# JunFenngZhi/YOLO-Fastest-and-Embedded-deployment

Measured on NVIDIA B200. Metric: images/sec at 640x512 b256, 1/2/4/8 B200; % HBM roofline per kernel, higher is better.
Workload: dtype f32

## Files before the change

### yolo_fastest_b200/csrc/yf_api.cu

```cuda
#include <cuda_runtime.h>

#include <algorithm>
#include <cmath>
#include <cstdarg>
#include <cstdio>
#include <cstdlib>
#include <cstring>
#include <map>
#include <string>
#include <utility>
#include <vector>

#include "../../include/yf.h"
#include "yf_kernels.cuh"
#include "yf_post.cuh"
#include "yf_tc.cuh"
#include "yf_tct.cuh"
#include "yf_wirb.cuh"
#include "yf_tcpw.cuh"
#include "yf_tcup.cuh"
#include "yf_tcirb2.cuh"
#include "yf_tcdense.cuh"
#include "yf_tcdense2.cuh"
#include "yf_prep.cuh"

using namespace yf;

namespace {

struct Spec {
    std::string name;
    int cin, cout, k, groups;
    bool deconv;
    int64_t w_off, b_off;
    int64_t w_count() const { return deconv ? (int64_t)cin * cout * k * k : (int64_t)cout * (cin / groups) * k * k; }
};

struct SpecTable {
    std::vector<Spec> specs;
    std::map<std::string, int> index;
    int64_t total = 0;
    void add(const std::string& name, int cin, int cout, int k, int groups = 1, bool deconv = false) {
        Spec s{name, cin, cout, k, groups, deconv, 0, 0};
        s.w_off = total;
        total += s.w_count();
        s.b_off = total;
        total += cout;
        index[name] = (int)specs.size();
        specs.push_back(s);
    }
    void irb(const std::string& name, int io, int mid) {
        add(name + ".conv1", io, mid, 1);
        add(name + ".conv2", mid, mid, 3, mid);
        add(name + ".conv3", mid, io, 1);
    }
    const Spec& get(const std::string& name) const { return specs[index.at(name)]; }
};

int head_channels(int num_cls, int num_anchors, int variant) {
    return (variant == YF_VARIANT_LITE ? num_anchors * num_cls : num_anchors) * (5 + num_cls);
}

SpecTable build_specs(int in_ch, int num_cls, int num_anchors, int variant = 0) {
    SpecTable t;
    const int nout = head_channels(num_cls, num_anchors, variant);
    t.add("conv0", in_ch, 8, 3);
    t.add("conv1_2", 8, 8, 1); t.add("conv1_3", 8, 8, 3, 8); t.add("conv1_4", 8, 4, 1);
    t.irb("res1_1", 4, 8);
    t.add("conv1_8", 4, 24, 1); t.add("conv1_9", 24, 24, 3); t.add("conv2_1", 24, 8, 1);
    t.irb("res2_1", 8, 32); t.irb("res2_2", 8, 32);
    t.add("conv2_2", 8, 32, 1); t.add("conv2_3", 32, 32, 3, 32); t.add("conv3_1", 32, 8, 1);
    t.irb("res3_1", 8, 48); t.irb("res3_2", 8, 48);
    t.add("conv3_2", 8, 48, 1); t.add("conv3_3", 48, 48, 3, 48); t.add("conv3_4", 48, 16, 1);
    t.irb("res3_3", 16, 96); t.irb("res3_4", 16, 96); t.irb("res3_5", 16, 96); t.irb("res3_6", 16, 96);
    t.add("conv3_5", 16, 96, 1); t.add("conv3_6", 96, 96, 3, 96); t.add("conv4_1", 96, 24, 1);
    t.irb("res4_1", 24, 136); t.irb("res4_2", 24, 136); t.irb("res4_3", 24, 136); t.irb("res4_4", 24, 136);
    t.add("conv4_2", 24, 136, 1); t.add("conv4_3", 136, 136, 3, 136); t.add("conv5_1", 136, 48, 1);
    t.irb("res5_1", 48, 224); t.irb("res5_2", 48, 224); t.irb("res5_3", 48, 224); t.irb("res5_4", 48, 224);
    t.irb("res5_5", 48, 224);
    t.add("conv5_2", 48, 96, 1);
    t.add("conv5_3", 96, 96, 5, 96); t.add("conv5_4", 96, 128, 1);
    t.add("conv5_5", 128, 128, 5, 128); t.add("conv5_6", 128, 128, 1);
    t.add("head_5", 128, nout, 1);
    t.add("deconv5_1", 96, 96, 2, 1, true);
    t.add("conv4_1_1", 232, 96, 1);
    t.add("conv4_1_2", 96, 96, 5, 96); t.add("conv4_1_3", 96, 96, 1);
    t.add("conv4_1_4", 96, 96, 5, 96); t.add("conv4_1_5", 96, 96, 1);
    t.add("head_4", 96, nout, 1);
    return t;
}

thread_local std::string g_err;

void set_err(std::string* dst, const char* fmt, ...) {
    char buf[1024];
    va_list ap;
    va_start(ap, fmt);
    vsnprintf(buf, sizeof buf, fmt, ap);
    va_end(ap);
    (dst ? *dst : g_err) = buf;
}

}

struct TmaCache {
    CUtensorMap map;
    const void* ptr = nullptr;
    int B = 0;
    bool u8 = false;
    bool failed = false;
};

struct GroupArgs {
    TmaCache* tc = nullptr;
    int nsm = 148;
    int resident = 148;
    const float* x = nullptr;
    const float* x2 = nullptr;
    float* y = nullptr;
    float* skip = nullptr;
    const float* w = nullptr;
    const float* w2 = nullptr;
    const DenseSmall* small = nullptr;
    bool pdl = false;
    int Hin = 0, Win = 0, Hout = 0, Wout = 0;
    int headn = 0;
};

template <class... KA, class... A>
inline void launch_k(bool pdl, void (*kernel)(KA...), int grid, int block, size_t smem, cudaStream_t st, A&&... args) {
    cudaLaunchConfig_t cfg;
    memset(&cfg, 0, sizeof cfg);
    cfg.gridDim = dim3((unsigned)grid); cfg.blockDim = dim3((unsigned)block); cfg.dynamicSmemBytes = smem; cfg.stream = st;
    cudaLaunchAttribute at[1];
    at[0].id = cudaLaunchAttributeProgrammaticStreamSerialization;
    at[0].val.programmaticStreamSerializationAllowed = 1;
    cfg.attrs = at; cfg.numAttrs = pdl ? 1u : 0u;
    cudaLaunchKernelEx(&cfg, kernel, std::forward<A>(args)...);
}

struct Group {
    int (*occupancy)() = nullptr;
    const char* name;
    void (*launch)(const GroupArgs&, const void* xin, bool u8in, int B, cudaStream_t);
    GroupArgs a;
    int out_ch;
    int64_t w_off;
    TmaCache tcache;
};

struct yf_ctx {
    int variant = 0;
    int device = 0, in_ch = 1, num_cls = 3, num_anchors = 3, max_batch = 1, H = 0, W = 0;
    int nout = 0;
    bool weights_loaded = false;
    std::string err;
    SpecTable specs;
    std::vector<Group> groups;
    std::vector<float> host_packed;
    float* d_w = nullptr;
    std::vector<float*> d_act;
    std::map<std::string, std::pair<float*, int64_t>> taps;
    float* d_skip = nullptr;
    float* d_hl = nullptr;
    float* d_hs = nullptr;
    float* d_x = nullptr;
    unsigned char* d_u8 = nullptr;
    yf_det* d_out = nullptr;
    int out_cap = 0;
    int32_t* d_counts = nullptr;
    int32_t* d_status = nullptr;
    int NC = 0;
    yf_det* p_rec = nullptr;
    double* p_conf = nullptr;
    int32_t* p_cls = nullptr;
    int4* p_sbox = nullptr;
    int32_t* p_order = nullptr;
    unsigned char* p_alive = nullptr;
    cudaStream_t s_copy = nullptr, s_comp = nullptr, s_back = nullptr;
    cudaStream_t s_cap = nullptr;
    cudaStream_t s_side = nullptr;
    DenseSmall dense_small;
    bool last_forward_forked = false;
    cudaEvent_t ev_fork = nullptr, ev_join = nullptr;
    unsigned char* sl_u8[2] = {nullptr, nullptr};
    yf_det* sl_out[2] = {nullptr, nullptr};
    int sl_out_cap[2] = {0, 0};
    int32_t* sl_counts[2] = {nullptr, nullptr};
    int32_t* sl_status[2] = {nullptr, nullptr};
    cudaEvent_t sl_in[2] = {nullptr, nullptr}, sl_free[2] = {nullptr, nullptr}, sl_done[2] = {nullptr, nullptr};
    bool sl_used[2] = {false, false};
    std::map<std::string, std::pair<cudaGraphExec_t, int>> graphs;
    PrepTap* prep_tab = nullptr;
    int prep_Ho = 0, prep_Wo = 0;
    unsigned char* d_bgr = nullptr;
    size_t bgr_cap = 0;
    unsigned char* n_alive = nullptr;
    int n_alive_cap = 0;
    int64_t launches = 0;
};

#define CTX_CHECK(ctx)                                         \
    if (!(ctx)) { set_err(nullptr, "null ctx"); return YF_ERR_ARG; }
#define CU(call)                                                                              \
    do {                                                                                      \
        cudaError_t e__ = (call);                                                             \
        if (e__ != cudaSuccess) {                                                             \
            set_err(&ctx->err, "%s failed: %s (%s:%d)", #call, cudaGetErrorString(e__), __FILE__, __LINE__); \
            return YF_ERR_CUDA;                                                               \
        }                                                                                     \
    } while (0)

#ifndef YF_CFGSTEM
#define YF_CFGSTEM StemCfg<8, 80, 256, 2>
#endif
using CfgStem = YF_CFGSTEM;
using CfgStem3 = StemCfg<8, 40, 256, 2, 3>;
#ifndef YF_CFGRES1
#define YF_CFGRES1 IrbCfg<4, 8, 4, 3, 1, 8, 80, 8, 8, 4, 8, 256, 3, true, true, false, false>
#endif
using CfgRes1 = YF_CFGRES1;
#ifndef YF_USE_WIRB
#define YF_USE_WIRB 1
#endif
#ifndef YF_CFGRES1_W
#define YF_CFGRES1_W WirbCfg<4, 8, 4, 1, 4, 8, 6, 12, true, true>
#endif
using CfgRes1W = YF_CFGRES1_W;
#ifndef YF_CFGRES2_W
#define YF_CFGRES2_W WirbCfg<8, 32, 8, 1, 8, 2, 6, 12, true, false>
#endif
using CfgRes2W = YF_CFGRES2_W;
#ifndef YF_CFGDOWN2_W
#define YF_CFGDOWN2_W WirbCfg<8, 32, 8, 2, 4, 2, 8, 12, false, false>
#endif
using CfgDown2W = YF_CFGDOWN2_W;
#ifndef YF_CFGSTEM_W
#define YF_CFGSTEM_W WstemCfg<12>
#endif
using CfgStemW = YF_CFGSTEM_W;

#ifndef YF_CFGDENSE
#define YF_CFGDENSE DenseCfg<8, 40, 4, 128, 3, 2>
#endif
using CfgDense = YF_CFGDENSE;
#ifndef YF_CFGRES2
#define YF_CFGRES2 IrbCfg<8, 32, 8, 3, 1, 8, 40, 16, 8, 4, 8, 128, 4, true, true, false, false>
#endif
using CfgRes2 = YF_CFGRES2;
#ifndef YF_CFGDOWN2
#define YF_CFGDOWN2 IrbCfg<8, 32, 8, 3, 2, 4, 40, 8, 8, 4, 4, 128, 3, true, false, false, false>
#endif
using CfgDown2 = YF_CFGDOWN2;
#ifndef YF_CFGRES3A
#define YF_CFGRES3A IrbCfg<8, 48, 8, 3, 1, 8, 40, 16, 8, 4, 8, 128, 4, true, true, false, false>
#endif
using CfgRes3a = YF_CFGRES3A;
#ifndef YF_CFGWIDE3
#define YF_CFGWIDE3 IrbCfg<8, 48, 16, 3, 1, 8, 40, 24, 8, 8, 8, 256, 2, true, false, false, false>
#endif
using CfgWide3 = YF_CFGWIDE3;
#ifndef YF_CFGRES3B
#define YF_CFGRES3B IrbCfg<16, 96, 16, 3, 1, 8, 40, 16, 8, 8, 8, 256, 2, true, true, false, false>
#endif
using CfgRes3b = YF_CFGRES3B;
#ifndef YF_TC3_TH
#define YF_TC3_TH 8
#define YF_TC3_TW 40
#define YF_TC3_MC 32
#define YF_TC3_RH 8
#define YF_TC3_NWW 10
#endif
#ifndef YF_TC3_OCC
#define YF_TC3_OCC 1
#endif
#ifndef YF_TC3_E1ALL
#define YF_TC3_E1ALL false
#endif
#ifndef YF_CFGRES3B_TC
#define YF_CFGRES3B_TC IrbTcCfg<16, 96, 16, YF_TC3_TH, YF_TC3_TW, YF_TC3_MC, YF_TC3_RH, YF_TC3_NWW, true, YF_TC3_E1ALL, YF_TC3_OCC>
#endif
using CfgRes3bTc = YF_CFGRES3B_TC;
#ifndef YF_USE_TCT
#define YF_USE_TCT 1
#endif
#ifndef YF_USE_TCT_A
#define YF_USE_TCT_A 1
#endif
using CfgRes3bTt = IrbTtCfg<16, 96, 16, 16, true>;
using CfgRes4Tt = IrbTtCfg<24, 136, 24, 8, true, 2>;
#ifndef YF_TCT_A_TH
#define YF_TCT_A_TH 16
#define YF_TCT_A_OCC 1
#endif
using CfgRes3aTt = IrbTtCfg<8, 48, 8, YF_TCT_A_TH, true, 0, YF_TCT_A_OCC>;
using CfgWide3Tt = IrbTtCfg<8, 48, 16, YF_TCT_A_TH, false, 0, YF_TCT_A_OCC>;
using CfgDown3Tt = IrbTtCfg<16, 96, 24, 8, false, 0, 1, 2>;
using CfgDown4Tt = IrbTtCfg<24, 136, 48, 4, false, 1, 1, 2, true, true>;
#ifndef YF_CFGRES4_TC
#define YF_CFGRES4_TC IrbTcCfg<24, 136, 24, 8, 20, 32, 4, 10, true, true>
#endif
using CfgRes4Tc = YF_CFGRES4_TC;
#ifndef YF_USE_TC
#define YF_USE_TC 1
#endif
#ifndef YF_CFGDOWN3
#define YF_CFGDOWN3 IrbCfg<16, 96, 24, 3, 2, 4, 40, 16, 8, 8, 4, 256, 2, true, false, false, false>
#endif
using CfgDown3 = YF_CFGDOWN3;
#ifndef YF_CFGRES4
#define YF_CFGRES4 IrbCfg<24, 136, 24, 3, 1, 8, 40, 16, 8, 8, 8, 256, 2, true, true, false, false>
#endif
using CfgRes4 = YF_CFGRES4;
#ifndef YF_CFGDOWN4
#define YF_CFGDOWN4 IrbCfg<24, 136, 48, 3, 2, 2, 20, 16, 8, 8, 2, 128, 4, true, false, true, true>
#endif
using CfgDown4 = YF_CFGDOWN4;
#ifndef YF_CFGRES5
#define YF_CFGRES5 IrbCfg<48, 224, 48, 3, 1, 8, 20, 16, 8, 8, 8, 256, 2, true, true, false, false>
#endif
using CfgRes5 = YF_CFGRES5;
#ifndef YF_CFGPW52
#define YF_CFGPW52 PwCfg<48, 96, 80, 8, 256, true>
#endif
using CfgPw52 = YF_CFGPW52;
using CfgLite34 = PwPwCfg<8, 48, 16, 128>;
#ifndef YF_CFGNECKS1
#define YF_CFGNECKS1 IrbCfg<96, 96, 128, 5, 1, 8, 20, 48, 4, 8, 4, 640, 1, false, false, false, false>
#endif
using CfgNeckS1 = YF_CFGNECKS1;
#ifndef YF_CFGNECKS2
#define YF_CFGNECKS2 IrbCfg<128, 128, 128, 5, 1, 8, 20, 32, 4, 8, 4, 640, 1, false, false, false, false, 1>
#endif
using CfgNeckS2 = YF_CFGNECKS2;
#ifndef YF_CFGUPCAT
#define YF_CFGUPCAT UpCatCfg<8, 20, 16, 4, 256, 2>
#endif
using CfgUpCat = YF_CFGUPCAT;
#ifndef YF_CFGNECKL1
#define YF_CFGNECKL1 IrbCfg<96, 96, 96, 5, 1, 4, 40, 32, 4, 8, 4, 256, 2, false, false, false, false>
#endif
using CfgNeckL1 = YF_CFGNECKL1;
#ifndef YF_CFGNECKL2
#define YF_CFGNECKL2 IrbCfg<96, 96, 96, 5, 1, 4, 40, 16, 4, 8, 4, 256, 2, false, false, false, false, 1>
#endif
using CfgNeckL2 = YF_CFGNECKL2;
#ifndef YF_CFGNECKS1_TC
#define YF_CFGNECKS1_TC DwPwTcCfg<96, 128, 5, 16, 20, 16, 4, 10, false>
#endif
using CfgNeckS1Tc = YF_CFGNECKS1_TC;
#ifndef YF_CFGNECKL1_TC
#define YF_CFGNECKL1_TC DwPwTcCfg<96, 96, 5, 8, 40, 16, 4, 10, false>
#endif
using CfgNeckL1Tc = YF_CFGNECKL1_TC;
#ifndef YF_CFGNECKS2_TC
#define YF_CFGNECKS2_TC DwPwTcCfg<128, 32, 5, 16, 20, 16, 4, 10, false, true>
#endif
using CfgNeckS2Tc = YF_CFGNECKS2_TC;
#ifndef YF_CFGNECKL2_TC
#define YF_CFGNECKL2_TC DwPwTcCfg<96, 32, 5, 8, 40, 16, 4, 10, false, true>
#endif
using CfgNeckL2Tc = YF_CFGNECKL2_TC;
static bool heads_on_tc(int nout) { return YF_USE_TC && nout <= 32; }
using CfgUpCatTc = UpCatTcCfg<10>;
using CfgDenseTc = DenseTcCfg<12>;
#ifndef YF_DENSE_TC
#define YF_DENSE_TC YF_USE_TC
#endif
#ifndef YF_RES5_TC
#define YF_RES5_TC YF_USE_TC
#endif
#ifndef YF_CFGRES5_TC
#define YF_CFGRES5_TC IrbTc2Cfg<48, 224, 48, 8, 20, 2, 2, 10, true>
#endif
using CfgRes5Tc = YF_CFGRES5_TC;
using CfgRes5TcS = IrbTc2Cfg<48, 224, 48, 4, 20, 2, 2, 10, true>;
using CfgRes4TcS = IrbTcCfg<24, 136, 24, 4, 20, 32, 4, 10, true, true>;
using CfgRes3bTcS = IrbTcCfg<16, 96, 16, 4, 40, 32, 4, 10, true, YF_TC3_E1ALL>;
using CfgRes5TcXS = IrbTc2Cfg<48, 224, 48, 2, 20, 2, 2, 10, true>;
using CfgRes5TcN = IrbTc2Cfg<48, 224, 48, 8, 12, 2, 2, 10, true>;
using CfgNeckS1TcN = DwPwTcCfg<96, 128, 5, 8, 12, 16, 4, 10, false>;
using CfgNeckS2TcN = DwPwTcCfg<128, 32, 5, 8, 12, 16, 4, 10, false, true>;
using CfgNeckL1TcN = DwPwTcCfg<96, 96, 5, 8, 20, 16, 4, 10, false>;
using CfgNeckL2TcN = DwPwTcCfg<96, 32, 5, 8, 20, 16, 4, 10, false, true>;
using CfgDown3N = IrbCfg<16, 96, 24, 3, 2, 4, 20, 16, 8, 8, 4, 256, 2, true, false, false, false>;
using CfgDown4N = IrbCfg<24, 136, 48, 3, 2, 2, 12, 16, 8, 8, 2, 128, 4, true, false, true, true>;
using CfgNeckL1TcS = DwPwTcCfg<96, 96, 5, 4, 20, 16, 4, 10, false>;
using CfgNeckL2TcS = DwPwTcCfg<96, 32, 5, 4, 20, 16, 4, 10, false, true>;
using CfgNeckS1TcS = DwPwTcCfg<96, 128, 5, 4, 20, 16, 4, 10, false>;
using CfgNeckS2TcS = DwPwTcCfg<128, 32, 5, 4, 20, 16, 4, 10, false, true>;
using CfgRes3bTcXS = IrbTcCfg<16, 96, 16, 2, 40, 32, 2, 10, true, YF_TC3_E1ALL>;
using CfgRes4TcXS = IrbTcCfg<24, 136, 24, 2, 20, 32, 2, 10, true, true>;
static bool upcat_on_tc(int H, int W) { return YF_USE_TC && ((W / 16) % 4 == 0) && ((H / 16) % 2 == 0); }

namespace {

template <class C>
void launch_irb(const GroupArgs& g, const void*, bool, int B, cudaStream_t st) {
    using G = typename C::G;
    const int tx = cdiv(g.Wout, G::TW), ty = cdiv(g.Hout, G::TH);
    const int total = B * tx * ty;
    const int grid = total < g.resident ? total : g.resident;
    irb_kernel<C><<<grid, C::NT, C::SMEM_BYTES, st>>>(g.x, g.y, g.skip, g.w, g.Hin, g.Win, g.Hout, g.Wout, tx, ty, total, g.headn);
}
template <class CB, class CN>
void launch_irb_auto(const GroupArgs& g, const void* x, bool u8, int B, cudaStream_t st) {
    static_assert(CB::CB == CN::CB && CB::OFF_B2 == CN::OFF_B2 && CB::MC == CN::MC, "both tile shapes read the same packed weights");
    const int big = B * cdiv(g.Wout, CB::G::TW) * cdiv(g.Hout, CB::G::TH);
    if (g.Wout <= CN::G::TW || 2 * big <= g.nsm) launch_irb<CN>(g, x, u8, B, st);
    else launch_irb<CB>(g, x, u8, B, st);
}
template <class K>
int occ_of(K kernel, int nt, int smem) {
    int n = 0;
    if (cudaOccupancyMaxActiveBlocksPerMultiprocessor(&n, kernel, nt, smem) != cudaSuccess || n < 1) n = 1;
    return n;
}
template <class C> int occ_irb() { return occ_of(irb_kernel<C>, C::NT, C::SMEM_BYTES); }
int occ_stem() { return occ_of(stem_kernel<CfgStem, false>, CfgStem::NT, CfgStem::SMEM_BYTES); }
int occ_stem3() { return occ_of(stem_kernel<CfgStem3, false>, CfgStem3::NT, CfgStem3::SMEM_BYTES); }
int occ_dense() { return occ_of(dense_kernel<CfgDense>, CfgDense::NT, CfgDense::SMEM_BYTES); }
int occ_upcat() { return occ_of(upcat_kernel<CfgUpCat>, CfgUpCat::NT, CfgUpCat::SMEM_BYTES); }
int occ_upcat_tc() { return occ_of(upcat_tc_kernel<CfgUpCatTc>, CfgUpCatTc::NT, CfgUpCatTc::SMEM_BYTES); }
void launch_upcat_tc(const GroupArgs& g, const void*, bool, int B, cudaStream_t st) {
    using C = CfgUpCatTc;
    const int tx = cdiv(g.Wout, C::TW), ty = cdiv(g.Hout, C::TH);
    const int total = B * tx * ty;
    const int grid = total < g.resident ? total : g.resident;
    launch_k(g.pdl, upcat_tc_kernel<C>, grid, C::NT, C::SMEM_BYTES, st, g.x, g.x2, g.y, g.w, g.Hout, g.Wout, tx, ty, total);
}

template <class C>
int wirb_band_rows(int B, int Hout, int Wout, int warps) {
    const int nstrips = cdiv(Wout, C::OW);
    long long best_cost = -1;
    int best_R = 1;
    for (int nch = 1; nch <= 16; ++nch) {
        const int R = C::S == 1 ? nch * C::RC - 2 : (nch * C::RC - 1) / 2;
        if (R < 1) continue;
        const long long units = (long long)B * nstrips * cdiv(Hout, R);
        const long long cost = ((units + warps - 1) / warps) * (nch * C::RC + 2);
        if (best_cost < 0 || cost <= best_cost) { best_cost = cost; best_R = R; }
        if (R >= Hout) break;
    }
    return best_R;
}
template <class C>
void launch_wirb(const GroupArgs& g, const void*, bool, int B, cudaStream_t st) {
    TmaCache* tc = g.tc;
    if (tc->ptr != g.x || tc->B != B) {
        tc->failed = tma_make_map4(&tc->map, g.x, 4, B, C::CIN, g.Hin, g.Win, C::XW, C::RC, C::CIN) != 0;
        tc->ptr = g.x; tc->B = B;
    }
    if (g.Wout % C::SPX) tc->failed = true;
    if (tc->failed) return;
    const int R = wirb_band_rows<C>(B, g.Hout, g.Wout, g.nsm * C::NW);
    const int nstrips = cdiv(g.Wout, C::OW), nbands = cdiv(g.Hout, R);
    const int total = B * nstrips * nbands;
    const int grid = std::min(g.nsm, cdiv(total, C::NW));
    launch_k(g.pdl, wirb_kernel<C>, grid, C::NW * 32, C::SMEM_BYTES, st, tc->map, g.y, g.w, g.Hin, g.Win, g.Hout, g.Wout, R, nstrips, nbands, total);
}
template <class C>
void launch_wstem(const GroupArgs& g, const void* xin, bool u8in, int B, cudaStream_t st) {
    TmaCache* tc = g.tc;
    if (tc->ptr != xin || tc->B != B || tc->u8 != u8in) {
        tc->failed = (u8in ? tma_make_map4(&tc->map, xin, 1, B, 1, g.Hin, g.Win, C::RAWWU, C::RAWH, 1)
                           : tma_make_map4(&tc->map, xin, 4, B, 1, g.Hin, g.Win, C::RAWW, C::RAWH, 1)) != 0;
        tc->ptr = xin; tc->B = B; tc->u8 = u8in;
    }
    if (g.Wout % C::SPX) tc->failed = true;
    if (tc->failed) return;
    const int R = wirb_band_rows<C>(B, g.Hout, g.Wout, g.nsm * C::NW);
    const int nstrips = cdiv(g.Wout, C::OW), nbands = cdiv(g.Hout, R);
    const int total = B * nstrips * nbands;
    const int grid = std::min(g.nsm, cdiv(total, C::NW));
    if (u8in) launch_k(g.pdl, wstem_kernel<C, true>, grid, C::NW * 32, C::template smem_bytes<true>(), st, tc->map, g.y, g.w, g.Hin, g.Win, g.Hout, g.Wout, R, nstrips, nbands, total);
    else launch_k(g.pdl, wstem_kernel<C, false>, grid, C::NW * 32, C::template smem_bytes<false>(), st, tc->map, g.y, g.w, g.Hin, g.Win, g.Hout, g.Wout, R, nstrips, nbands, total);
}
template <class C>
cudaError_t init_wstem() {
    cudaError_t e = cudaFuncSetAttribute(wstem_kernel<C, true>, cudaFuncAttributeMaxDynamicSharedMemorySize, C::template smem_bytes<true>());
    if (e != cudaSuccess) return e;
    return cudaFuncSetAttribute(wstem_kernel<C, false>, cudaFuncAttributeMaxDynamicSharedMemorySize, C::template smem_bytes<false>());
}

template <class C>
cudaError_t init_wirb() { return cudaFuncSetAttribute(wirb_kernel<C>, cudaFuncAttributeMaxDynamicSharedMemorySize, C::SMEM_BYTES); }

template <class C>
void launch_dwpwtc(const GroupArgs& g, const void*, bool, int B, cudaStream_t st) {
    using G = typename C::G;
    const int tx = cdiv(g.Wout, G::TW), ty = cdiv(g.Hout, G::TH);
    const int total = B * tx * ty;
    const int grid = total < g.resident ? total : g.resident;
    launch_k(g.pdl, dwpw_tc_kernel<C>, grid, C::NT, C::SMEM_BYTES, st, g.x, g.y, g.w, g.Hout, g.Wout, tx, ty, total, g.headn > 0 ? g.headn : C::N);
}
template <class CB, class CS, class CN>
void launch_dwpwtc_auto(const GroupArgs& g, const void* x, bool u8, int B, cudaStream_t st) {
    static_assert(CB::WFLOATS == CS::WFLOATS && CB::CB == CS::CB && CB::WFLOATS == CN::WFLOATS && CB::CB == CN::CB, "all tile shapes read the same packed weights");
    const int big = B * cdiv(g.Wout, CB::G::TW) * cdiv(g.Hout, CB::G::TH);
    if (g.Wout <= CN::G::TW) launch_dwpwtc<CN>(g, x, u8, B, st);
    else if (2 * big <= g.nsm) launch_dwpwtc<CS>(g, x, u8, B, st);
    else launch_dwpwtc<CB>(g, x, u8, B, st);
}
template <class C> int occ_dwpwtc() { return occ_of(dwpw_tc_kernel<C>, C::NT, C::SMEM_BYTES); }
template <class C>
cudaError_t init_dwpwtc() { return cudaFuncSetAttribute(dwpw_tc_kernel<C>, cudaFuncAttributeMaxDynamicSharedMemorySize, C::SMEM_BYTES); }

template <class C>
void launch_irbtc2(const GroupArgs& g, const void*, bool, int B, cudaStream_t st) {
    using G = typename C::G;
    const int tx = cdiv(g.Wout, G::TW), ty = cdiv(g.Hout, G::TH);
    const int total = B * tx * ty;
    const int grid = total < g.resident ? total : g.resident;
    launch_k(g.pdl, irbtc2_kernel<C>, grid, C::NT, C::SMEM_BYTES, st, g.x, g.y, g.w, g.Hout, g.Wout, tx, ty, total);
}
template <class CB, class CS>
void launch_irbtc2_auto(const GroupArgs& g, const void* x, bool u8, int B, cudaStream_t st) {
    const int big = B * cdiv(g.Wout, CB::G::TW) * cdiv(g.Hout, CB::G::TH);
    if (g.Wout <= CfgRes5TcN::G::TW) launch_irbtc2<CfgRes5TcN>(g, x, u8, B, st);
    else if (4 * big <= g.nsm) launch_irbtc2<CfgRes5TcXS>(g, x, u8, B, st);
    else if (2 * big <= g.nsm) launch_irbtc2<CS>(g, x, u8, B, st);
    else launch_irbtc2<CB>(g, x, u8, B, st);
}
template <class C> int occ_irbtc2() { return occ_of(irbtc2_kernel<C>, C::NT, C::SMEM_BYTES); }
template <class C>
cudaError_t init_irbtc2() { return cudaFuncSetAttribute(irbtc2_kernel<C>, cudaFuncAttributeMaxDynamicSharedMemorySize, C::SMEM_BYTES); }

template <class C>
void launch_irbtc(const GroupArgs& g, const void*, bool, int B, cudaStream_t st) {
    using G = typename C::G;
    const int tx = cdiv(g.Wout, G::TW), ty = cdiv(g.Hout, G::TH);
    const int total = B * tx * ty;
    const int grid = total < g.resident ? total : g.resident;
    irbtc_kernel<C><<<grid, C::NT, C::SMEM_BYTES, st>>>(g.x, g.y, g.w, g.Hout, g.Wout, tx, ty, total);
}
template <class CB, class CS, class CXS>
void launch_irbtc_auto(const GroupArgs& g, const void* x, bool u8, int B, cudaStream_t st) {
    static_assert(CB::WFLOATS == CS::WFLOATS && CB::CB == CS::CB && CB::OFF_B2 == CS::OFF_B2 && CB::WFLOATS == CXS::WFLOATS && CB::CB == CXS::CB,
                  "all tile shapes read the same packed weights");
    const int big = B * cdiv(g.Wout, CB::G::TW) * cdiv(g.Hout, CB::G::TH);
    if (4 * big <= g.nsm) launch_irbtc<CXS>(g, x, u8, B, st);
    else if (2 * big <= g.nsm) launch_irbtc<CS>(g, x, u8, B, st);
    else launch_irbtc<CB>(g, x, u8, B, st);
}
template <class C>
void launch_irbt(const GroupArgs& g, const void*, bool, int B, cudaStream_t st, int64_t w_off = 0) {
    TmaCache* tc = g.tc;
    if (tc->ptr != g.x || tc->B != B) {
        tc->failed = tma_make_map4(&tc->map, g.x, 4, B, C::CIN, g.Hin, g.Win, C::RW, C::HR, C::CIN) != 0;
        tc->ptr = g.x; tc->B = B;
    }
    if (tc->failed) return;
    const int tx = cdiv(g.Wout, C::TW), ty = cdiv(g.Hout, C::TH);
    const int total = B * tx * ty;
    const int grid = total < g.nsm * C::OCC ? total : g.nsm * C::OCC;
    launch_k(g.pdl, irbt_kernel<C>, grid, C::NT, C::SMEM_BYTES, st, tc->map, g.x, g.y, g.skip, g.w + w_off, g.Hin, g.Win, g.Hout, g.Wout, tx, ty, total);
}
template <class C>
cudaError_t init_irbt() { return cudaFuncSetAttribute(irbt_kernel<C>, cudaFuncAttributeMaxDynamicSharedMemorySize, C::SMEM_BYTES); }
template <class C> void launch_irbt0(const GroupArgs& g, const void* x, bool u8, int B, cudaStream_t st) { launch_irbt<C>(g, x, u8, B, st, 0); }
template <class CT, class CB, class CS, class CXS>
void launch_res4_auto(const GroupArgs& g, const void* x, bool u8, int B, cudaStream_t st) {
    if (g.Wout % 4 == 0) launch_irbt<CT>(g, x, u8, B, st, g.w2 - g.w);
    else launch_irbtc_auto<CB, CS, CXS>(g, x, u8, B, st);
}
template <class CT, class CB, class CN>
void launch_down4_auto(const GroupArgs& g, const void* x, bool u8, int B, cudaStream_t st) {
    if (g.Win % 4 == 0) launch_irbt<CT>(g, x, u8, B, st, g.w2 - g.w);
    else launch_irb_auto<CB, CN>(g, x, u8, B, st);
}
template <class C> int occ_irbt() { return occ_of(irbt_kernel<C>, C::NT, C::SMEM_BYTES); }
template <class C> int occ_irbtc() { return occ_of(irbtc_kernel<C>, C::NT, C::SMEM_BYTES); }
template <class C>
cudaError_t init_irbtc() { return cudaFuncSetAttribute(irbtc_kernel<C>, cudaFuncAttributeMaxDynamicSharedMemorySize, C::SMEM_BYTES); }

template <class C>
cudaError_t init_irb() { return cudaFuncSetAttribute(irb_kernel<C>, cudaFuncAttributeMaxDynamicSharedMemorySize, C::SMEM_BYTES); }

template <class C>
void launch_stem(const GroupArgs& g, const void* xin, bool u8in, int B, cudaStream_t st) {
    using G = typename C::G;
    const int tx = cdiv(g.Wout, G::TW), ty = cdiv(g.Hout, G::TH);
    const int total = B * tx * ty;
    const int grid = total < g.resident ? total : g.resident;
    if (u8in) stem_kernel<C, true><<<grid, C::NT, C::SMEM_BYTES, st>>>(xin, g.y, g.w, g.Hin, g.Win, g.Hout, g.Wout, tx, ty, total);
    else stem_kernel<C, false><<<grid, C::NT, C::SMEM_BYTES, st>>>(xin, g.y, g.w, g.Hin, g.Win, g.Hout, g.Wout, tx, ty, total);
}
int occ_dense_tc() { return occ_of(dense_tc_kernel<CfgDenseTc>, CfgDenseTc::NT, CfgDenseTc::SMEM_BYTES); }
void launch_dense_tc(const GroupArgs& g, const void*, bool, int B, cudaStream_t st) {
    using C = CfgDenseTc;
    const int tx = cdiv(g.Wout, C::TW), ty = cdiv(g.Hout, C::TH);
    const int total = B * tx * ty;
    const int grid = total < g.resident ? total : g.resident;
    launch_k(g.pdl, dense_tc_kernel<C>, grid, C::NT, C::SMEM_BYTES, st, g.x, g.y, g.w, g.Hin, g.Win, g.Hout, g.Wout, tx, ty, total);
}
#ifndef YF_DENSE_TA
#define YF_DENSE_TA 1
#endif
int occ_dense_ta() { return occ_of(dense_ta_kernel<DenseTaCfg>, DenseTaCfg::NT, DenseTaCfg::SMEM_BYTES); }
void launch_dense_ta(const GroupArgs& g, const void*, bool, int B, cudaStream_t st) {
    using C = DenseTaCfg;
    TmaCache* tc = g.tc;
    if (tc->ptr != g.x || tc->B != B) {
        tc->failed = tma_make_map4(&tc->map, g.x, 4, B, 4, g.Hin, g.Win, C::XW, C::RH, 4) != 0;
        tc->ptr = g.x; tc->B = B;
    }
    if (tc->failed) return;
    const int tx = cdiv(g.Wout, C::TW), ty = cdiv(g.Hout, C::TH);
    const int total = B * tx * ty;
    const int grid = total < g.resident ? total : g.resident;
    launch_k(g.pdl, dense_ta_kernel<C>, grid, C::NT, C::SMEM_BYTES, st, tc->map, g.y, g.w, *g.small, g.Hin, g.Win, g.Hout, g.Wout, tx, ty, total);
}
void launch_dense(const GroupArgs& g, const void*, bool, int B, cudaStream_t st) {
    using C = CfgDense;
    using G = C::G;
    const int tx = cdiv(g.Wout, G::TW), ty = cdiv(g.Hout, G::TH);
    const int total = B * tx * ty;
    const int grid = total < g.resident ? total : g.resident;
    dense_kernel<C><<<grid, C::NT, C::SMEM_BYTES, st>>>(g.x, g.y, g.w, g.Hin, g.Win, g.Hout, g.Wout, tx, ty, total);
}
void launch_pw52(const GroupArgs& g, const void*, bool, int B, cudaStream_t st) {
    using C = CfgPw52;
    const int HW = g.Hin * g.Win;
    const int tiles = cdiv(HW, C::PIXT);
    launch_k(g.pdl, pw_kernel<C>, B * tiles, C::NT, C::SMEM_BYTES, st, g.x, g.y, g.w, HW, tiles);
}
void launch_lite34(const GroupArgs& g, const void*, bool, int B, cudaStream_t st) {
    using C = CfgLite34;
    const int HW = g.Hin * g.Win;
    const long long groups = (long long)B * (HW / 4);
    const int grid = (int)std::min<long long>((groups + C::NT - 1) / C::NT, (long long)g.nsm * 8);
    pwpw_kernel<C><<<grid, C::NT, 0, st>>>(g.x, g.y, g.w, HW, groups);
}
void launch_upcat(const GroupArgs& g, const void*, bool, int B, cudaStream_t st) {
    using C = CfgUpCat;
    const int tx = cdiv(g.Wout, C::TW), ty = cdiv(g.Hout, C::TH);
    const int total = B * tx * ty;
    const int grid = total < g.resident ? total : g.resident;
    upcat_kernel<C><<<grid, C::NT, C::SMEM_BYTES, st>>>(g.x, g.x2, g.y, g.w, g.Hout, g.Wout, tx, ty, total);
}

struct Folded {
    const float* blob;
    const SpecTable* t;
    const float* w(const std::string& n) const { return blob + t->get(n).w_off; }
    const float* b(const std::string& n) const { return blob + t->get(n).b_off; }
};

void pad4(std::vector<float>& v) { while (v.size() % 4) v.push_back(0.f); }

template <class C>
int64_t pack_irb(std::vector<float>& out, const Folded& f, const std::string& n1, const std::string& nd,
                 const std::string& n2, const std::string& nh, int headn) {
    pad4(out);
    const int64_t off = (int64_t)out.size();
    const int headp = rup(headn, 4);
    out.resize(off + (C::HEADC ? C::OFF_WH + C::CMIDP * headp + headp : C::OFF_B2 + C::COUT), 0.f);
    float* o = out.data() + off;
    for (int c = 0; c < C::NCHUNK; ++c) {
        float* cb = o + (int64_t)c * C::CB;
        for (int ml = 0; ml < C::MC; ++ml) {
            const int m = c * C::MC + ml;
            if (m >= C::CMID) continue;
            if (C::EXPAND) {
                for (int k = 0; k < C::CIN; ++k) cb[C::OFF_W1 + k * C::MC + ml] = f.w(n1)[m * C::CIN + k];
                cb[C::OFF_B1 + ml] = f.b(n1)[m];
            }
            for (int t = 0; t < C::KK; ++t) cb[C::OFF_WD + ml * C::KK + t] = f.w(nd)[m * C::KK + t];
            cb[C::OFF_BD + ml] = f.b(nd)[m];
            if (!C::HEADC)
                for (int n = 0; n < C::COUT; ++n) cb[C::OFF_W2 + ml * C::COUT + n] = f.w(n2)[n * C::CMID + m];
        }
    }
    if (!C::HEADC) {
        for (int n = 0; n < C::COUT; ++n) o[C::OFF_B2 + n] = f.b(n2)[n];
    } else {
        float* wh = o + C::OFF_WH;
        float* bh = wh + C::CMIDP * headp;
        for (int n = 0; n < headn; ++n) {
            for (int m = 0; m < C::CMID; ++m) {
                double a = 0.0;
                for (int k = 0; k < C::COUT; ++k) a += (double)f.w(nh)[n * C::COUT + k] * (double)f.w(n2)[k * C::CMID + m];
                wh[m * headp + n] = (float)a;
            }
            double b = (double)f.b(nh)[n];
            for (int k = 0; k < C::COUT; ++k) b += (double)f.w(nh)[n * C::COUT + k] * (double)f.b(n2)[k];
            bh[n] = (float)b;
        }
    }
    return off;
}

inline float tf32_rna_host(float v) {
    uint32_t u;
    memcpy(&u, &v, 4);
    u = (u + 0x1000u) & 0xFFFFE000u;
    memcpy(&v, &u, 4);
    return v;
}
inline void put_kmajor_split(float* hi, float* lo, int n, int k, int K, float w) {
    const int idx = ((n >> 3) * (K / 4) + (k >> 2)) * 32 + (n & 7) * 4 + (k & 3);
    const float h = tf32_rna_host(w);
    hi[idx] = h;
    lo[idx] = tf32_rna_host(w - h);
}

template <class C>
int64_t pack_wirb(std::vector<float>& out, const Folded& f, const std::string& n1, const std::string& nd, const std::string& n2) {
    pad4(out);
    const int64_t off = (int64_t)out.size();
    out.resize(off + C::WFLOATS, 0.f);
    float* o = out.data() + off;
    for (int m = 0; m < C::CMID; ++m) {
        for (int k = 0; k < C::CIN; ++k) o[C::OFF_W1 + k * C::CMID + m] = f.w(n1)[m * C::CIN + k];
        o[C::OFF_B1 + m] = f.b(n1)[m];
        for (int t = 0; t < 9; ++t) o[C::OFF_WD + t * C::CMID + m] = f.w(nd)[m * 9 + t];
        o[C::OFF_BD + m] = f.b(nd)[m];
        for (int n = 0; n < C::COUT; ++n) o[C::OFF_W2 + n * C::CMID + m] = f.w(n2)[n * C::CMID + m];
    }
    for (int n = 0; n < C::COUT; ++n) o[C::OFF_B2 + n] = f.b(n2)[n];
    return off;
}

template <class C>
int64_t pack_dwpwtc_head(std::vector<float>& out, const Folded& f, const std::string& nd, const std::string& n2, const std::string& nh, int mid, int headn) {
    pad4(out);
    while (out.size() % 32) out.push_back(0.f);
    const int64_t off = (int64_t)out.size();
    out.resize(off + C::WFLOATS, 0.f);
    float* o = out.data() + off;
    for (int c = 0; c < C::NCHUNK; ++c) {
        float* cb = o + (int64_t)c * C::CB;
        for (int ml = 0; ml < C::MC; ++ml) {
            const int m = c * C::MC + ml;
            for (int t = 0; t < C::KK; ++t) cb[C::OFF_WD + ml * C::KK + t] = f.w(nd)[m * C::KK + t];
            cb[C::OFF_BD + ml] = f.b(nd)[m];
            for (int n = 0; n < headn; ++n) {
                double a = 0.0;
                for (int k = 0; k < mid; ++k) a += (double)f.w(nh)[n * mid + k] * (double)f.w(n2)[k * C::C + m];
                put_kmajor_split(cb + C::OFF_WH, cb + C::OFF_WL, n, ml, C::MC, (float)a);
            }
        }
    }
    for (int n = 0; n < headn; ++n) {
        double b = (double)f.b(nh)[n];
        for (int k = 0; k < mid; ++k) b += (double)f.w(nh)[n * mid + k] * (double)f.b(n2)[k];
        o[C::OFF_B + n] = (float)b;
    }
    return off;
}

int64_t pack_upcat_tc(std::vector<float>& out, const Folded& f) {
    using C = CfgUpCatTc;
    pad4(out);
    while (out.size() % 32) out.push_back(0.f);
    const int64_t off = (int64_t)out.size();
    out.resize(off + C::WFLOATS, 0.f);
    float* o = out.data() + off;
    const float* w = f.w("conv4_1_1");
    const float* wt = f.w("deconv5_1");
    int slot = 0;
    auto a_steps = [&](int h) {
        for (int kc = 0; kc < C::NKA; ++kc, ++slot) {
            float* sb = o + (int64_t)slot * C::SLOT;
            for (int par = 0; par < 4; ++par)
                for (int ml = 0; ml < 48; ++ml)
                    for (int kl = 0; kl < C::MC; ++kl) {
                        const int c = kc * C::MC + kl, m = 48 * h + ml;
                        put_kmajor_split(sb, sb + C::NHALF * C::MC, par * 48 + ml, kl, C::MC, wt[((c * 96 + m) * 2 + (par >> 1)) * 2 + (par & 1)]);
                    }
        }
    };
    auto b_step = [&](int k0, int kvalid) {
        float* sb = o + (int64_t)slot * C::SLOT;
        for (int n = 0; n < C::N; ++n)
            for (int kl = 0; kl < kvalid; ++kl) put_kmajor_split(sb, sb + C::N * C::MC, n, kl, C::MC, w[n * 232 + k0 + kl]);
        ++slot;
    };
    a_steps(0);
    for (int c = 0; c < C::NSKIP; ++c) b_step(c * C::MC, std::min(C::MC, C::CS - c * C::MC));
    for (int j = 0; j < C::NUPH; ++j) b_step(C::CS + j * C::MC, C::MC);
    a_steps(1);
    for (int j = 0; j < C::NUPH; ++j) b_step(C::CS + 48 + j * C::MC, C::MC);
    for (int m = 0; m < 96; ++m) o[C::OFF_BT + m] = f.b("deconv5_1")[m];
    for (int n = 0; n < 96; ++n) o[C::OFF_B + n] = f.b("conv4_1_1")[n];
    return off;
}

template <class C>
int64_t pack_irbtc2(std::vector<float>& out, const Folded& f, const std::string& n1, const std::string& nd, const std::string& n2) {
    pad4(out);
    while (out.size() % 32) out.push_back(0.f);
    const int64_t off = (int64_t)out.size();
    out.resize(off + C::WFLOATS, 0.f);
    float* o = out.data() + off;
    int slot = 0;
    for (int h = 0; h < C::NH; ++h) {
        for (int kc = 0; kc < C::NKA; ++kc, ++slot) {
            float* sb = o + (int64_t)slot * C::SLOT;
            for (int ml = 0; ml < C::NA; ++ml) {
                const int m = h * C::NA + ml;
                if (m >= C::CMID) continue;
                for (int kl = 0; kl < C::MC; ++kl) put_kmajor_split(sb, sb + C::NA * C::MC, ml, kl, C::MC, f.w(n1)[m * C::CIN + kc * C::MC + kl]);
            }
        }
        for (int j = 0; j < C::NMC; ++j, ++slot) {
            float* sb = o + (int64_t)slot * C::SLOT;
            for (int ml = 0; ml < C::MC; ++ml) {
                const int m = h * C::NA + j * C::MC + ml;
// ... 1242 lines not shown
```

Measured before the change: 52960.

## Add TMA-fed warp-specialized pipeline for fused depthwise+pointwise tensor-core kernel

Adds a new dwpw kernel variant in which a dedicated producer warp loads input halo boxes through a TMA tensor map into a multi-stage shared-memory ring. Compute warps run the 5x5 depthwise stage and feed double-buffered TF32 operands to a tcgen05 MMA warp, which accumulates into double-buffered TMEM. The epilogue for one tile overlaps the depthwise work for the next. The path is on by default when the output width is a multiple of 4 and falls back to the old kernel otherwise. In exchange it uses more shared memory and a map-caching scheme keyed on pointer, batch and box.

```diff
diff --git a/yolo_fastest_b200/csrc/yf_api.cu b/yolo_fastest_b200/csrc/yf_api.cu
--- a/yolo_fastest_b200/csrc/yf_api.cu
+++ b/yolo_fastest_b200/csrc/yf_api.cu
@@ -18,6 +18,7 @@
 #include "yf_tct.cuh"
 #include "yf_wirb.cuh"
 #include "yf_tcpw.cuh"
+#include "yf_tcpw_tma.cuh"
 #include "yf_tcup.cuh"
 #include "yf_tcirb2.cuh"
 #include "yf_tcdense.cuh"
@@ -108,6 +109,7 @@
     const void* ptr = nullptr;
     int B = 0;
     bool u8 = false;
+    int box = 0;
     bool failed = false;
 };
 
@@ -487,13 +489,29 @@
 template <class C>
 cudaError_t init_wirb() { return cudaFuncSetAttribute(wirb_kernel<C>, cudaFuncAttributeMaxDynamicSharedMemorySize, C::SMEM_BYTES); }
 
+#ifndef YF_DWPW_TMA
+#define YF_DWPW_TMA 1
+#endif
 template <class C>
 void launch_dwpwtc(const GroupArgs& g, const void*, bool, int B, cudaStream_t st) {
     using G = typename C::G;
+    using T = DwPwTmaCfg<C>;
     const int tx = cdiv(g.Wout, G::TW), ty = cdiv(g.Hout, G::TH);
     const int total = B * tx * ty;
     const int grid = total < g.resident ? total : g.resident;
-    launch_k(g.pdl, dwpw_tc_kernel<C>, grid, C::NT, C::SMEM_BYTES, st, g.x, g.y, g.w, g.Hout, g.Wout, tx, ty, total, g.headn > 0 ? g.headn : C::N);
+    const int nout = g.headn > 0 ? g.headn : C::N;
+    bool tma = YF_DWPW_TMA && g.Wout % 4 == 0;
+    if (tma) {
+        TmaCache* tc = g.tc;
+        const int box = T::BW * 1024 + T::BH;
+        if (tc->ptr != g.x || tc->B != B || (tc->box != box && tc->box != -box)) {
+            const bool ok = tma_make_map4(&tc->map, g.x, 4, B, C::C, g.Hout, g.Wout, T::BW, T::BH, C::MC) == 0;
+            tc->ptr = g.x; tc->B = B; tc->box = ok ? box : -box;
+        }
+        tma = tc->box == box;
+    }
+    if (tma) launch_k(g.pdl, dwpw_tma_kernel<T>, grid, T::NT, T::SMEM_BYTES, st, g.tc->map, g.y, g.w, g.Hout, g.Wout, tx, ty, total, nout);
+    else launch_k(g.pdl, dwpw_tc_kernel<C>, grid, C::NT, C::SMEM_BYTES, st, g.x, g.y, g.w, g.Hout, g.Wout, tx, ty, total, nout);
 }
 template <class CB, class CS, class CN>
 void launch_dwpwtc_auto(const GroupArgs& g, const void* x, bool u8, int B, cudaStream_t st) {
@@ -503,9 +521,15 @@
     else if (2 * big <= g.nsm) launch_dwpwtc<CS>(g, x, u8, B, st);
     else launch_dwpwtc<CB>(g, x, u8, B, st);
 }
-template <class C> int occ_dwpwtc() { return occ_of(dwpw_tc_kernel<C>, C::NT, C::SMEM_BYTES); }
-template <class C>
-cudaError_t init_dwpwtc() { return cudaFuncSetAttribute(dwpw_tc_kernel<C>, cudaFuncAttributeMaxDynamicSharedMemorySize, C::SMEM_BYTES); }
+template <class C> int occ_dwpwtc() {
+    return std::min(occ_of(dwpw_tc_kernel<C>, C::NT, C::SMEM_BYTES), occ_of(dwpw_tma_kernel<DwPwTmaCfg<C>>, DwPwTmaCfg<C>::NT, DwPwTmaCfg<C>::SMEM_BYTES));
+}
+template <class C>
+cudaError_t init_dwpwtc() {
+    const cudaError_t e = cudaFuncSetAttribute(dwpw_tc_kernel<C>, cudaFuncAttributeMaxDynamicSharedMemorySize, C::SMEM_BYTES);
+    if (e != cudaSuccess) return e;
+    return cudaFuncSetAttribute(dwpw_tma_kernel<DwPwTmaCfg<C>>, cudaFuncAttributeMaxDynamicSharedMemorySize, DwPwTmaCfg<C>::SMEM_BYTES);
+}
 
 template <class C>
 void launch_irbtc2(const GroupArgs& g, const void*, bool, int B, cudaStream_t st) {
diff --git a/yolo_fastest_b200/csrc/yf_tcpw_tma.cuh b/yolo_fastest_b200/csrc/yf_tcpw_tma.cuh
--- /dev/null
+++ b/yolo_fastest_b200/csrc/yf_tcpw_tma.cuh
@@ -0,0 +1,244 @@
+#pragma once
+#include "yf_tcpw.cuh"
+#include "yf_tma.cuh"
+
+namespace yf {
+
+constexpr int dwpw_tma_rh(int TH, int TW, int MC, int NTW) {
+    for (int rh = 8; rh > 1; rh >>= 1)
+        if (TH % rh == 0 && MC * (TH / rh) * (TW / 2) >= NTW) return rh;
+    return 1;
+}
+
+template <class B>
+struct DwPwTmaCfg : B {
+    using G = typename B::G;
+    static constexpr int MC = B::MC, NTW = B::NTW, NWB = B::NWB, CB = B::CB, DA1 = B::DA1, MT3 = B::MT3, NP = B::NP;
+    static constexpr int NT = NTW + 64;
+    static constexpr int BW = G::TW + 8, BH = G::IH;
+    static constexpr int BOX = MC * BH * BW;
+    static constexpr int RH = dwpw_tma_rh(G::TH, G::TW, MC, NTW);
+    static constexpr int ACOLS = pow2_ge(MT3 * NP);
+    static constexpr int NACC = 2 * ACOLS <= 512 ? 2 : 1;
+    static constexpr int TCOLS = NACC * ACOLS;
+    static constexpr int FIXED = 4 * DA1 + NWB * CB;
+    static constexpr int NST = (FIXED + 3 * BOX) * 4 + 1024 <= 227 * 1024 ? 3 : 2;
+    static constexpr int SMEM_BYTES = (FIXED + NST * BOX) * 4 + 1024;
+    static_assert(G::KS == 5 && G::S == 1 && G::P == 2, "5x5 stride 1: the box starts 2 columns left of the halo");
+    static_assert(G::TW % 4 == 0 && BW <= 256 && BH <= 256 && MC <= 256, "TMA box dimensions");
+    static_assert((BOX * 4) % 128 == 0 && (CB * 4) % 128 == 0, "ring stages stay 128-byte aligned");
+    static_assert(SMEM_BYTES <= 227 * 1024, "two ring stages do not fit shared memory");
+    static_assert(BOX * 4 >= 4096, "over-read guard behind the operand regions");
+    static_assert(G::TH % RH == 0, "row strips");
+};
+
+template <class C>
+__device__ __forceinline__ void dwk_tma_stage(int tid, const float* __restrict__ Xb, const float* __restrict__ Wd, const float* __restrict__ bd,
+                                              float* __restrict__ DAhi, float* __restrict__ DAlo) {
+    using G = typename C::G;
+    constexpr int RH = C::RH, NSTRIP = G::TW / 2, NSEG = G::TH / RH, NITEM = C::MC * NSEG * NSTRIP;
+    for (int item = tid; item < NITEM; item += C::NTW) {
+        const int g = item % NSTRIP, rest = item / NSTRIP;
+        const int seg = rest % NSEG, m = rest / NSEG;
+        float w[25];
+#pragma unroll
+        for (int t = 0; t < 25; ++t) w[t] = Wd[m * 25 + t];
+        const float b = bd[m];
+        const float* e = Xb + m * C::BH * C::BW + (seg * RH) * C::BW + 2 * g + 2;
+        float2 win[5][5];
+        auto load_row = [&](float2 (&r)[5], const float* p) {
+            const float2 a = *reinterpret_cast<const float2*>(p);
+            const float2 c = *reinterpret_cast<const float2*>(p + 2);
+            const float2 d = *reinterpret_cast<const float2*>(p + 4);
+            r[0] = a; r[1] = make_float2(a.y, c.x); r[2] = c; r[3] = make_float2(c.y, d.x); r[4] = d;
+        };
+#pragma unroll
+        for (int dd = 0; dd < 4; ++dd) load_row(win[dd + 1], e + dd * C::BW);
+#pragma unroll
+        for (int oy = 0; oy < RH; ++oy) {
+#pragma unroll
+            for (int dd = 0; dd < 4; ++dd)
+#pragma unroll
+                for (int v = 0; v < 5; ++v) win[dd][v] = win[dd + 1][v];
+            load_row(win[4], e + (oy + 4) * C::BW);
+            float2 a = make_float2(b, b);
+#pragma unroll
+            for (int dy = 0; dy < 5; ++dy)
+#pragma unroll
+                for (int dx = 0; dx < 5; ++dx) a = __ffma2_rn(make_float2(w[dy * 5 + dx], w[dy * 5 + dx]), win[dy][dx], a);
+            const float v0 = fmaxf(a.x, 0.f), v1 = fmaxf(a.y, 0.f);
+            const float h0 = tf32_hi(v0), h1 = tf32_hi(v1);
+            const int o = a_idx((seg * RH + oy) * G::TW + 2 * g, m, C::KB3);
+            *reinterpret_cast<float2*>(DAhi + o) = make_float2(h0, h1);
+            *reinterpret_cast<float2*>(DAlo + o) = make_float2(v0 - h0, v1 - h1);
+        }
+    }
+}
+
+template <class C>
+__global__ void __launch_bounds__(C::NT, 1)
+dwpw_tma_kernel(const __grid_constant__ CUtensorMap xmap, float* __restrict__ y, const float* __restrict__ wts, int H, int W,
+                int tiles_x, int tiles_y, int total_tiles, int nout ) {
+    using G = typename C::G;
+    constexpr int NWW = C::NWW, NCH = C::NCHUNK, NST = C::NST, NACC = C::NACC;
+    extern __shared__ unsigned char smem_raw[];
+    float* base = reinterpret_cast<float*>(smem_raw + ((1024u - (smem_u32(smem_raw) & 1023u)) & 1023u));
+    float* Dbuf = base;
+    float* Xb = Dbuf + 4 * C::DA1;
+    float* Ws = Xb + NST * C::BOX;
+    __shared__ __align__(8) uint64_t wbar[C::NWB], xfull[NST], xfree[NST], dfull[2], dfree[2], ofull[NACC], ofree[NACC];
+    __shared__ uint32_t tmem_slot;
+    const int tid = threadIdx.x, warp = tid >> 5, lane = tid & 31;
+
+    if (tid == 0) {
+        for (int i = 0; i < C::NWB; ++i) mbar_init(&wbar[i], 1);
+        for (int i = 0; i < NST; ++i) { mbar_init(&xfull[i], 1); mbar_init(&xfree[i], NWW); }
+        for (int i = 0; i < 2; ++i) { mbar_init(&dfull[i], NWW); mbar_init(&dfree[i], 1); }
+        for (int i = 0; i < NACC; ++i) { mbar_init(&ofull[i], 1); mbar_init(&ofree[i], NWW); }
+        mbar_fence_init();
+    }
+    if (warp == NWW) {
+        asm volatile("tcgen05.alloc.cta_group::1.sync.aligned.shared::cta.b32 [%0], %1;" ::"r"(smem_u32(&tmem_slot)), "r"((uint32_t)C::TCOLS) : "memory");
+        asm volatile("tcgen05.relinquish_alloc_permit.cta_group::1.sync.aligned;" ::: "memory");
+    }
+    if (warp == NWW + 1) tma_prefetch_desc(&xmap);
+    tc_fence_before();
+    __syncthreads();
+    tc_fence_after();
+    pdl_trigger();
+    pdl_wait();
+    const uint32_t tmem = tmem_slot;
+
+    const int ntile = total_tiles > (int)blockIdx.x ? (total_tiles - (int)blockIdx.x + (int)gridDim.x - 1) / (int)gridDim.x : 0;
+    const int S = ntile * NCH;
+    const int tpi = tiles_x * tiles_y;
+    const uint32_t inv_tx = (65536u + (uint32_t)tiles_x - 1u) / (uint32_t)tiles_x;
+    auto origin = [&](int ti, int& b, int& oy0, int& ox0) {
+        const int tile = (int)blockIdx.x + ti * (int)gridDim.x;
+        b = tile / tpi;
+        const int t = tile - b * tpi;
+        const int ty = (int)(((uint32_t)t * inv_tx) >> 16);
+        oy0 = ty * G::TH; ox0 = (t - ty * tiles_x) * G::TW;
+    };
+
+    if (warp == NWW) {
+        if (S > 0 && elect_one()) {
+            constexpr uint32_t IDESC = umma_idesc_tf32(C::NP);
+            const uint32_t ws = smem_u32(Ws);
+            auto issue_w = [&](int q) {
+                const int slot = q % C::NWB;
+                mbar_expect_tx(&wbar[slot], C::CB * 4);
+                bulk_load(Ws + slot * C::CB, wts + (size_t)(q % NCH) * C::CB, C::CB * 4, &wbar[slot]);
+            };
+            const uint64_t dd0 = umma_desc(smem_u32(Dbuf), 1024, 512, 1);
+            const uint64_t dw0 = umma_desc(ws, 128, (C::MC / 4) * 128, 0);
+            issue_w(0);
+            if (S > 1) issue_w(1);
+            for (int q = 0; q < S; ++q) {
+                const int b = q & 1, c = q % NCH, ti = q / NCH, ab = ti % NACC;
+                if (c == 0 && ti >= NACC) mbar_wait(&ofree[ab], ((ti / NACC) - 1) & 1);
+                mbar_wait(&dfull[b], (q >> 1) & 1);
+                mbar_wait(&wbar[q % C::NWB], (q / C::NWB) & 1);
+                tc_fence_after();
+                const uint64_t wb = dw0 + (uint64_t)(((uint32_t)(q % C::NWB) * C::CB * 4) >> 4);
+                const uint64_t db = dd0 + (uint64_t)((uint32_t)(b * 2 * C::DA1 * 4) >> 4);
+                const uint32_t acc = tmem + (uint32_t)(ab * C::ACOLS);
+#pragma unroll 1
+                for (int mt = 0; mt < C::MT3; ++mt) {
+                    const uint64_t mo = (uint64_t)(mt * 256);
+#pragma unroll
+                    for (int pass = 0; pass < 3; ++pass) {
+#pragma unroll
+                        for (int kb = 0; kb < C::MC / 8; ++kb)
+                            umma_tf32(acc + mt * C::NP, db + mo + (uint64_t)(((pass == 2 ? C::DA1 : 0) + kb * C::KB3) * 4 / 16),
+                                      wb + (uint64_t)(((pass == 1 ? C::OFF_WL : C::OFF_WH) * 4 + kb * 256) / 16), IDESC,
+                                      (c | pass | kb) ? 1u : 0u);
+                    }
+                }
+                umma_commit(&dfree[b]);
+                if (c == NCH - 1) umma_commit(&ofull[ab]);
+                if (q + 2 < S) {
+                    if (q >= 1) mbar_wait(&dfree[(q - 1) & 1], ((q - 1) >> 1) & 1);
+                    issue_w(q + 2);
+                }
+            }
+        }
+    } else if (warp == NWW + 1) {
+        if (S > 0 && elect_one()) {
+            int q = 0;
+            for (int ti = 0; ti < ntile; ++ti) {
+                int b, oy0, ox0;
+                origin(ti, b, oy0, ox0);
+#pragma unroll 1
+                for (int c = 0; c < NCH; ++c, ++q) {
+                    const int st = q % NST;
+                    if (q >= NST) mbar_wait(&xfree[st], ((q / NST) - 1) & 1);
+                    mbar_expect_tx(&xfull[st], C::BOX * 4);
+                    tma_load4(Xb + st * C::BOX, &xmap, &xfull[st], ox0 - 4, oy0 - G::P, c * C::MC, b);
+                }
+            }
+        }
+    } else {
+        const int quarter = warp & 3, wq = warp >> 2;
+        const int nwq = (NWW - quarter + 3) >> 2;
+        const uint32_t lane_base = (uint32_t)(quarter * 32) << 16;
+        const size_t plane = (size_t)H * W;
+        auto epilogue = [&](int ti) {
+            int tb, oy0, ox0;
+            origin(ti, tb, oy0, ox0);
+            const int ab = ti % NACC;
+            mbar_wait(&ofull[ab], (ti / NACC) & 1);
+            tc_fence_after();
+            for (int u = wq; u < C::MT3 * (C::NP / 16); u += nwq) {
+                const int mt = u / (C::NP / 16), c0 = (u - mt * (C::NP / 16)) * 16;
+                if (mt * 128 + quarter * 32 >= G::OPIX) break;
+                const int pix = mt * 128 + quarter * 32 + lane;
+                const int oy = pix / G::TW, ox = pix - oy * G::TW;
+                const int gy = oy0 + oy, gx = ox0 + ox;
+                float v[16];
+                tmem_ld16(tmem + lane_base + (uint32_t)(ab * C::ACOLS) + mt * C::NP + c0, v);
+                if (pix < G::OPIX && gy < H && gx < W) {
+                    const int nch = C::NRT ? nout : C::N;
+                    float* yp = y + ((size_t)tb * nch + c0) * plane + (size_t)gy * W + gx;
+#pragma unroll
+                    for (int i = 0; i < 16; ++i) {
+                        if (c0 + i < nch) {
+                            float r = v[i] + __ldg(wts + C::OFF_B + c0 + i);
+                            if (C::RELU) r = fmaxf(r, 0.f);
+                            yp[i * plane] = r;
+                        }
+                    }
+                }
+            }
+            tc_fence_before();
+            __syncwarp();
+            if (lane == 0) mbar_arrive(&ofree[ab]);
+        };
+
+        int q = 0;
+        for (int ti = 0; ti < ntile; ++ti) {
+#pragma unroll 1
+            for (int c = 0; c < NCH; ++c, ++q) {
+                const int b = q & 1, st = q % NST;
+                const float* Wc = Ws + (q % C::NWB) * C::CB;
+                mbar_wait(&xfull[st], (q / NST) & 1);
+                mbar_wait(&wbar[q % C::NWB], (q / C::NWB) & 1);
+                if (q >= 2) mbar_wait(&dfree[b], ((q >> 1) - 1) & 1);
+                float* Dh = Dbuf + b * 2 * C::DA1;
+                dwk_tma_stage<C>(tid, Xb + st * C::BOX, Wc + C::OFF_WD, Wc + C::OFF_BD, Dh, Dh + C::DA1);
+                fence_proxy_async();
+                __syncwarp();
+                if (lane == 0) { mbar_arrive(&xfree[st]); mbar_arrive(&dfull[b]); }
+                if (c == 0 && ti > 0) epilogue(ti - 1);
+            }
+        }
+        if (ntile > 0) epilogue(ntile - 1);
+    }
+    __syncthreads();
+    if (warp == NWW) {
+        __syncwarp();
+        asm volatile("tcgen05.dealloc.cta_group::1.sync.aligned.b32 %0, %1;" ::"r"(tmem), "r"((uint32_t)C::TCOLS) : "memory");
+    }
+}
+
+}
```

Result: faster. 54590 (median of 6 runs) (+3.1%).
